# LuoGroup2023/PanTax

Measured on AMD Instinct MI355X. Metric: PAO wall-time (s) + Mreads/s: packed reads + DB (graphs and their unique-trio index) resident in HBM -> abundance tables; the metric's own GAF -> abundance quantity is value_gaf_to_tables (files -> tables, never `value`), higher is better.
Workload: dtype int64+f64

## Files before the change

### pantax_amd/csrc/api_core.cpp

```cpp
#include <algorithm>
#include <chrono>
#include <cstdio>
#include <cstdlib>
#include <cstring>
#include <memory>
#include <numeric>
#include <string>
#include "common.hpp"

using namespace ptx;

extern "C" {

int pantax_hip_db_upload(pantax_hip_ctx *ctx, const pantax_hip_graphs *g, pantax_hip_db **out) {
    if (!ctx || !g || !out) return PANTAX_HIP_E_INVALID;
    *out = nullptr;
    PTX_ENTER(ctx);
    uint32_t S = g->n_species;
    if (S == 0) return fail(ctx, PANTAX_HIP_E_INVALID, "db_upload: n_species == 0");
    std::unique_ptr<pantax_hip_db> db(new pantax_hip_db());
    db->S = S;
    if (!g->node_len) {
        std::vector<uint32_t> order(S), rs(S), re(S);
        std::iota(order.begin(), order.end(), 0u);
        std::stable_sort(order.begin(), order.end(), [&](uint32_t a, uint32_t b) { return g->range_start[a] < g->range_start[b]; });
        bool disjoint = true;
        for (uint32_t i = 0; i < S; ++i)
            if (g->range_start[i] < 0 || g->range_end[i] > 0xFFFFFFFFll) return fail(ctx, PANTAX_HIP_E_INVALID, "db_upload: species %u has an invalid node id range", i);
        for (uint32_t i = 0; i + 1 < S; ++i) if (g->range_end[order[i]] >= g->range_start[order[i + 1]]) disjoint = false;
        db->ranges_sorted_disjoint = disjoint;
        if (!disjoint) std::iota(order.begin(), order.end(), 0u);
        for (uint32_t i = 0; i < S; ++i) { rs[i] = (uint32_t)g->range_start[order[i]]; re[i] = (uint32_t)g->range_end[order[i]]; }
        db->h_range_start.assign(g->range_start, g->range_start + S);
        db->h_range_end.assign(g->range_end, g->range_end + S);
        PTX_TRY(upload(ctx, db->d_rng_start, rs.data(), S));
        PTX_TRY(upload(ctx, db->d_rng_end, re.data(), S));
        PTX_TRY(upload(ctx, db->d_rng_idx, order.data(), S));
        PTX_HIP(ctx, hipStreamSynchronize(ctx->stream));
        *out = db.release();
        return 0;
    }
// ... 196 lines not shown
        }
    }
    PTX_HIP(ctx, hipStreamSynchronize(stream));
    return 0;
}

int db_upload_finish(Ctx *ctx, pantax_hip_db *db_raw) {
    Db *const db = db_raw;
    const uint32_t S = db->S;
    const bool trace = ctx->cfg.trace;
    auto t_prev = std::chrono::steady_clock::now();
    auto lap = [&](const char *what) {
        if (!trace) return;
        (void)hipStreamSynchronize(ctx->stream);
        const auto now = std::chrono::steady_clock::now();
        std::fprintf(stderr, "[db_upload]            %-28s %9.3f ms\n", what, std::chrono::duration<double, std::milli>(now - t_prev).count());
        t_prev = now;
    };
    {
        DevBuf<uint32_t> d_flags;
        PTX_HIP(ctx, d_flags.alloc(2));
        PTX_HIP(ctx, hipMemsetAsync(d_flags.p, 0, sizeof(uint32_t), ctx->stream));
        PTX_HIP(ctx, hipMemsetAsync(d_flags.p + 1, 0xFF, sizeof(uint32_t), ctx->stream));
        PTX_TRY(node_tables_launch(ctx, db, d_flags.p));
        uint32_t fl[2] = {0, 0};
        uint64_t L = 0;
        PTX_TRY(download(ctx, fl, d_flags.p, 2));
        PTX_TRY(download(ctx, &L, db->d_bit_off.p + db->V, 1));
        PTX_TRY(download(ctx, db->h_all_same.data(), db->d_all_same.p, S));
        PTX_HIP(ctx, hipStreamSynchronize(ctx->stream));
        if (fl[0]) return fail(ctx, PANTAX_HIP_E_INVALID, "db_upload: a graph holds a node of length 0 (reference asserts > 0, profile.rs:494)");
        if (fl[1] != 0xFFFFFFFFu) return fail(ctx, PANTAX_HIP_E_INVALID, "db_upload: hap %u walks a node outside its species graph", fl[1] - 1);
        db->L = L;
        if (db->L >= NODE_REC_MAX_BITS) return fail(ctx, PANTAX_HIP_E_LIMIT, "db_upload: %llu graph bases on one GPU (limit 2^40)", (unsigned long long)db->L);
    }
    lap("node tables + checks (device)");
    {
        std::vector<uint2> tiles;
        constexpr uint64_t XCD = 8;
        for (uint32_t s = 0; s < S; ++s) {
            uint64_t maxlen = 0;
            for (uint64_t h = db->h_hap_off[s]; h < db->h_hap_off[s + 1]; ++h) maxlen = std::max<uint64_t>(maxlen, db->h_path_off[h + 1] - db->h_path_off[h]);
            const uint64_t n_chunks = (maxlen + PATH_TILE - 1) / PATH_TILE;
            for (uint64_t c0 = 0; c0 < n_chunks; c0 += XCD) {
                while (tiles.size() % XCD) tiles.push_back(make_uint2(0xFFFFFFFFu, 0u));
                for (uint64_t h = db->h_hap_off[s]; h < db->h_hap_off[s + 1]; ++h)
                    for (uint64_t c = c0; c < c0 + XCD; ++c) {
                        const bool live = c < n_chunks && c * PATH_TILE < db->h_path_off[h + 1] - db->h_path_off[h];
                        tiles.push_back(live ? make_uint2((uint32_t)h, (uint32_t)c) : make_uint2(0xFFFFFFFFu, 0u));
                    }
            }
        }
        db->n_tiles = tiles.size();
        PTX_TRY(upload(ctx, db->d_tiles, tiles.data(), tiles.size()));
        std::vector<uint32_t> hap_tile_off(db->H + 1, 0), tile_rank(tiles.size());
        for (uint64_t h = 0; h < db->H; ++h)
            hap_tile_off[h + 1] = hap_tile_off[h] + (uint32_t)((db->h_path_off[h + 1] - db->h_path_off[h] + PATH_TILE - 1) / PATH_TILE);
        for (size_t i = 0; i < tiles.size(); ++i) tile_rank[i] = tiles[i].x == 0xFFFFFFFFu ? hap_tile_off[db->H] : hap_tile_off[tiles[i].x] + tiles[i].y;
        PTX_TRY(upload(ctx, db->d_tile_rank, tile_rank.data(), tile_rank.size()));
        PTX_TRY(upload(ctx, db->d_hap_tile_off, hap_tile_off.data(), hap_tile_off.size()));
    }
    {
        const uint64_t TILE = 2048, nt = (db->V + TILE - 1) / TILE;
        std::vector<uint2> tsp(nt ? nt : 1, make_uint2(0u, 0u));
        uint32_t sp = 0;
        for (uint64_t t = 0; t < nt; ++t) {
// ... 136 lines not shown
```

### pantax_amd/csrc/common.hpp

```cpp
#pragma once
#include <hip/hip_runtime.h>
#include <cstdint>
#include <cstdio>
#include <map>
#include <functional>
#include <mutex>
#include <cstring>
#include <atomic>
#include <string>
#include <vector>
#include "../../include/pantax_hip.h"
#include "cov_state.hpp"
#include "reads_state.hpp"
#include "upload_host.hpp"

#ifndef TRIO_LH_PACK
#define TRIO_LH_PACK 0
#endif
namespace ptx {

struct Ctx;
#if TRIO_LH_PACK
using trio_len_t = uint2;
#else
// ... 255 lines not shown
    DevBuf<uint32_t> d_counts;
    uint32_t k_cap = 0;
    DevBuf<uint64_t> d_pat_mask;
    DevBuf<uint32_t> d_pat_start;
    DevBuf<uint32_t> d_pat_species;
    DevBuf<uint32_t> d_sp_pat_off;
    std::vector<uint32_t> h_sp_pat_off;
    LadPatScratch pat_scratch;
    DevBuf<double> d_x, d_x2, d_obj, d_obj2;
    DevBuf<int32_t> d_status, d_iters, d_status2, d_iters2;
    DevBuf<uint8_t> d_fixed2, d_need2;
};


struct TrioScratch {
    DevBuf<uint32_t> zero_arena;
    DevBuf<uint32_t> cnt, cursor, bucket_off, scan_tmp, first_cnt, d_tot;
    DevBuf<uint4> bucket;
    DevBuf<uint32_t> uniq_q;
    DevBuf<uint32_t> row_q;
    DevBuf<uint64_t> vis_uq;
    DevBuf<uint4> vis_rec;
    DevBuf<uint32_t> gprefix;
    uint32_t gprefix_for = 0;
    DevBuf<uint32_t> group_sums;
    DevBuf<uint32_t> hap_cnt;
};

inline uint64_t next_db_uid() { static std::atomic<uint64_t> n{1}; return n.fetch_add(1); }
struct Db {
    const uint64_t uid = next_db_uid();
    uint32_t S = 0;
    uint64_t V = 0, H = 0, P = 0, L = 0;
    std::vector<int64_t> h_range_start, h_range_end;
    std::vector<uint64_t> h_node_off, h_hap_off, h_path_off;
    bool ranges_sorted_disjoint = true;
    DevBuf<uint32_t> d_rng_start, d_rng_end, d_rng_idx;
    DevBuf<uint32_t> d_sp_first_id;
    DevBuf<uint32_t> d_node_base;
    DevBuf<uint64_t> d_bit_off;
    DevBuf<uint32_t> d_node_len;
    DevBuf<uint4> d_node_rec;
    DevBuf<uint64_t> d_path_off;
    DevBuf<uint32_t> d_path_nodes;
    DevBuf<uint32_t> d_hap_species;
    DevBuf<uint64_t> d_hap_off;
    DevBuf<uint8_t> d_all_same;
    std::vector<uint8_t> h_all_same;
    DevBuf<uint2> d_tiles;
    uint64_t n_tiles = 0;
    DevBuf<uint2> d_emit_tile_sp;
    DevBuf<uint64_t> d_node_haps;
    bool nh_built = false, nh_walk_too = false;
    DevBuf<uint32_t> d_tile_rank;
    DevBuf<uint32_t> d_hap_tile_off;
    bool trio_visit_ok = false;
    uint32_t n_vgroups = 0;
    std::vector<uint8_t> h_trio_slow;
    DevBuf<uint32_t> d_trio_slow;
    DevBuf<uint32_t> d_vis_pos;
    DevBuf<uint64_t> d_vis_head;
    DevBuf<uint32_t> d_vis_nbase;
    DevBuf<uint32_t> d_vis_sp;
    DevBuf<uint32_t> d_node_visited;
    bool trio_block_ok = false;
    uint32_t n_blocks = 0;
// ... 111 lines not shown
__host__ __device__ inline uint32_t nr_filter(uint32_t y) { return y >> 24; }
__host__ __device__ inline uint32_t nr_head(uint32_t y_old, uint32_t rows, uint32_t filter) { return (y_old & 0xFFu) | ((rows & 0xFFFFu) << 8) | (filter << 24); }
__host__ __device__ inline uint32_t nr_pair_bit(uint32_t lo, uint32_t hi) { return 1u << (((lo * 0x9E3779B1u) ^ (hi * 0x85EBCA77u)) >> 29); }
__host__ __device__ inline uint64_t nr_bit_off(const uint4 &r) { return ((uint64_t)(r.y & 0xFFu) << 32) | r.x; }
__host__ __device__ inline uint4 nr_make(uint64_t bit_off, uint32_t len) { return make_uint4((uint32_t)bit_off, (uint32_t)(bit_off >> 32) & 0xFFu, len, 0u); }

template <class T>
int upload(Ctx *ctx, DevBuf<T> &dst, const T *src, size_t n) {
    PTX_HIP(ctx, dst.alloc(n));
    if (n) PTX_HIP(ctx, hipMemcpyAsync(dst.p, src, n * sizeof(T), hipMemcpyHostToDevice, ctx->stream));
    return 0;
}
int upload_segments(Ctx *ctx, void *d_dst, const UploadSeg *segs, size_t n_segs, const std::string *files, int64_t *bad_seg, hipStream_t stream = nullptr );

constexpr uint32_t PK_BLOCK = 256, PK_UNIT = 256;
struct PackedWalks {
    uint64_t n_blocks = 0, payload_bytes = 0;
    UploadSeg first_seg, off_seg, payload_seg;
};
struct GraphPart {
    uint64_t n_nodes = 0, n_haps = 0;
    const uint64_t *path_off = nullptr;
    UploadSeg len_seg;
    bool len16 = false;
    std::vector<UploadSeg> walk_segs;
    bool packed = false;
    PackedWalks pk;
};
struct UnpackSpecies { uint32_t blk_base, off_base, payload_base , out_base, n_steps, payload_units ; };
int walks_unpack_launch(Ctx *ctx, const UnpackSpecies *d_table, uint32_t n_species, uint32_t n_blocks, const uint32_t *d_first, const uint32_t *d_off,
                        const uint8_t *d_payload, uint32_t *d_path_nodes, hipStream_t stream = nullptr );
struct WidenSpecies { uint64_t src_base , dst_base; uint64_t n; };
int lens_widen_launch(Ctx *ctx, const WidenSpecies *d_table, uint32_t n_species, uint64_t n_total, const uint16_t *d_len16, uint32_t *d_node_len, hipStream_t stream = nullptr);
int node_tables_launch(Ctx *ctx, Db *db, uint32_t *d_flags );
int db_upload_parts(Ctx *ctx, uint32_t S, const int64_t *range_start, const int64_t *range_end, const GraphPart *parts, const std::string *files,
                    pantax_hip_db **out);
int db_upload_begin(Ctx *ctx, uint32_t S, const int64_t *range_start, const int64_t *range_end, const GraphPart *parts, pantax_hip_db **out);
int db_upload_arrays(Ctx *ctx, pantax_hip_db *db, const GraphPart *parts, const std::string *files, hipStream_t stream);
int db_upload_finish(Ctx *ctx, pantax_hip_db *db);
int upload_big(Ctx *ctx, void *d_dst, const void *src, uint64_t bytes);
int upload_file(Ctx *ctx, void *d_dst, int fd, uint64_t file_off, uint64_t bytes);
int upload_text_pieces(Ctx *ctx, size_t n_pieces, void *const *d_dst, const char *text, int fd, uint64_t file_base, const uint64_t *piece_off, const uint64_t *piece_end,
                       hipStream_t stream, const std::function<bool(size_t)> &before_piece, const std::function<int(size_t)> &after_piece);
constexpr size_t PIN_UP_RING = 1u << 20, PIN_UP_MAX = 1u << 16;
template <class T>
int upload_small(Ctx *ctx, DevBuf<T> &dst, const T *src, size_t n) {
    const size_t bytes = n * sizeof(T);
    if (bytes == 0 || bytes > PIN_UP_MAX) return upload(ctx, dst, src, n);
    PTX_HIP(ctx, dst.alloc(n));
    PTX_HIP(ctx, ctx->pin_up.reserve(PIN_UP_RING));
    size_t off = (ctx->pin_up_off + 63) & ~(size_t)63;
    constexpr size_t HALF = PIN_UP_RING / 2;
    const int h_old = ctx->pin_up_off ? (int)((ctx->pin_up_off - 1) / HALF) : 0;
    if (off < HALF && off + bytes > HALF) off = HALF;
    if (off + bytes > PIN_UP_RING) off = 0;
    const int h_new = off >= HALF ? 1 : 0;
    if (h_new != h_old) {
        for (int k = 0; k < 2; ++k) {
            hipStream_t st = k == 0 ? (ctx->stream_main ? ctx->stream_main : ctx->stream) : ctx->stream2;
            if (!st) continue;
            if (!ctx->pin_up_ev[h_old][k]) PTX_HIP(ctx, hipEventCreateWithFlags(&ctx->pin_up_ev[h_old][k], hipEventDisableTiming));
            PTX_HIP(ctx, hipEventRecord(ctx->pin_up_ev[h_old][k], st));
        }
        ctx->pin_up_ev_set[h_old] = true;
        if (ctx->pin_up_ev_set[h_new])
            for (int k = 0; k < 2; ++k) if (ctx->pin_up_ev[h_new][k]) PTX_HIP(ctx, hipEventSynchronize(ctx->pin_up_ev[h_new][k]));
// ... 102 lines not shown
```

### pantax_amd/csrc/ssn_node_pass.hip

```cpp
#include <type_traits>
#include "ssn_device.hpp"

namespace ptx {

namespace {
template <bool HAPS>
__global__ void __launch_bounds__(256) ssn_hist_kernel(Sn sn) {
    __shared__ ulonglong2 tree[SN_NLEAF];
    __shared__ uint32_t s_hist[SN_NBUCKET];
    extern __shared__ unsigned long long s_dyn_tab[];
    __shared__ int s_bit[64];
    __shared__ unsigned long long s_acc[2 * 64];
    const uint32_t s = blockIdx.y, g = blockIdx.x, o = sn.node_base[s], n = sn.node_base[s + 1] - o;
    uint32_t *w = sn.w(s);
    if (n == 0 || w[SN_OFF_FLAGS] != 0) return;
    if (HAPS && sn.skip_empty && sn.hp.sp_p[s] <= 0) {
        uint32_t *row0 = sn.cntm + ((size_t)s * sn.G + g) * SN_NBUCKET;
        for (int i = threadIdx.x; i < SN_NBUCKET; i += 256) row0[i] = 0u;
        if (threadIdx.x == 0) { sn.stage_cnt[(size_t)s * sn.G + g] = 0u; if (sn.c0) sn.c0p[(size_t)s * sn.G + g] = 0.0; }
        return;
    }
    uint32_t t0, t1;
    sn_tiles(sn, n, g, t0, t1);
    const ulonglong2 *gt = reinterpret_cast<const ulonglong2 *>(w + SN_OFF_TREE);
// ... 95 lines not shown
        }
    }
    __syncthreads();
    uint32_t *row = sn.cntm + ((size_t)s * sn.G + g) * SN_NBUCKET;
    for (int i = threadIdx.x; i < SN_NBUCKET; i += 256) row[i] = s_hist[i];
    if (threadIdx.x == 0) sn.stage_cnt[(size_t)s * sn.G + g] = s_nstage;
    if (sn.c0) {
        __shared__ double s_c[4];
        cacc = wave_reduce(cacc, [](double x, double y) { return x + y; });
        if (lane == 0) s_c[threadIdx.x >> 6] = cacc;
        __syncthreads();
        if (threadIdx.x == 0) sn.c0p[(size_t)s * sn.G + g] = (s_c[0] + s_c[1]) + (s_c[2] + s_c[3]);
    }
    if (HAPS && p0 > 0 && sn.hp.ratio) {
#pragma unroll
        for (int k = 0; k < 8; ++k) {
            if (k >= p0) break;
            const unsigned long long cs = wave_reduce(c8[k], [](unsigned long long x, unsigned long long y) { return x + y; });
            const unsigned long long ls = wave_reduce(l8[k], [](unsigned long long x, unsigned long long y) { return x + y; });
            if (lane == 0) {
                if (cs) atomicAdd(&s_acc[2 * k], cs);
                if (ls) atomicAdd(&s_acc[2 * k + 1], ls);
            }
        }
        __syncthreads();
        if ((int)threadIdx.x < 2 * p0 && s_acc[threadIdx.x]) atomicAdd(&sn.hp.ratio[2 * h0 + threadIdx.x], s_acc[threadIdx.x]);
    }
}

constexpr int SN_HALF = SN_ITEMS >= 8 ? SN_ITEMS / 2 : SN_ITEMS;
static_assert(SN_ITEMS % SN_HALF == 0, "whole halves");
constexpr int SN_HALVES = SN_ITEMS / SN_HALF;
static_assert(2 * SN_HALF <= 64, "a lane per end of the half's items");
template <int NB>
__global__ void __launch_bounds__(256) node_rows_kernel(Sn sn) {
    __shared__ ulonglong2 tree[SN_NLEAF];
    __shared__ uint32_t s_hist[SN_NBUCKET];
    extern __shared__ unsigned long long s_dyn_tab[];
    __shared__ int s_bit[64];
    __shared__ unsigned long long s_acc[2 * 64];
    const uint32_t s = blockIdx.y, g = blockIdx.x, o = sn.node_base[s], n = sn.node_base[s + 1] - o;
    uint32_t *w = sn.w(s);
    if (n == 0 || w[SN_OFF_FLAGS] != 0) return;
    uint32_t t0, t1;
    sn_tiles(sn, n, g, t0, t1);
    if (sn.skip_empty && sn.hp.sp_p[s] <= 0) {
        uint32_t *row0 = sn.cntm + ((size_t)s * sn.G + g) * SN_NBUCKET;
        for (int i = threadIdx.x; i < SN_NBUCKET; i += 256) row0[i] = 0u;
        if (threadIdx.x == 0) { sn.stage_cnt[(size_t)s * sn.G + g] = 0u; if (sn.c0) sn.c0p[(size_t)s * sn.G + g] = 0.0; }
        if (!sn.fz.active || sn.fz.active[s]) {
            NodeAcc acc;
            for (uint32_t t = t0; t < t1; ++t)
#pragma unroll
                for (int r = 0; r < SN_ITEMS; ++r) {
                    const uint32_t i = t * SN_TILE + (uint32_t)r * 256u + threadIdx.x;
                    if (i < n) acc.add((double)(long long)sn.fz.bases[o + i] / (double)sn.hp.node_len[o + i], sn.fz.min_depth);
                }
            sn_block_partial<4>(acc, sn.npart + (size_t)s * sn.G + g);
        }
        return;
    }
    const ulonglong2 *gt = reinterpret_cast<const ulonglong2 *>(w + SN_OFF_TREE);
    __shared__ uint32_t s_nstage;
    const int lane = threadIdx.x & 63;
    const uint32_t wave64 = (uint32_t)__builtin_amdgcn_readfirstlane((int)(threadIdx.x >> 6)) << 6;
    constexpr int HALF = SN_HALF;
    auto end_of = [&](uint32_t q) -> uint64_t {
        const uint32_t i = q * (uint32_t)(HALF * 256) + (uint32_t)((lane >> 1) % HALF) * 256u + wave64 + (uint32_t)(lane & 1) * 64u;
        return sn.fz.bit_off[o + (i < n ? i : n)];
    };
    uint64_t endv = 0;
    if (NB && t0 < t1) endv = end_of(t0 * (uint32_t)SN_HALVES);
    for (int i = threadIdx.x; i < SN_NBUCKET; i += 256) s_hist[i] = 0;
    if (threadIdx.x == 0) s_nstage = 0;
    if (t0 < t1) for (int i = threadIdx.x; i < SN_NLEAF; i += 256) tree[i] = gt[i];
    const uint64_t h0 = sn.hp.hap_off[s], nh = sn.hp.hap_off[s + 1] - h0;
    int p0 = sn.hp.sp_p[s];
    if (p0 <= 0 || p0 > 64 || nh > 64) p0 = 0;
    const int nbyte = p0 ? (int)((nh + 7) / 8) : 0;
    if (threadIdx.x < 64) s_bit[threadIdx.x] = (p0 && threadIdx.x < nh) ? sn.hp.hap_bit[h0 + threadIdx.x] : -1;
    if (threadIdx.x < 128) s_acc[threadIdx.x] = 0;
    __syncthreads();
    for (int b = 0; b < nbyte; ++b) {
        unsigned long long e = 0ull;
#pragma unroll
        for (int i = 0; i < 8; ++i) { const int bit = s_bit[8 * b + i]; if (((threadIdx.x >> i) & 1u) && bit >= 0) e |= 1ull << bit; }
        s_dyn_tab[b * 256 + threadIdx.x] = e;
    }
    __syncthreads();
    uint64_t eb[2 * HALF];
#pragma unroll
    for (int k = 0; k < 2 * HALF; ++k) eb[k] = NB ? lane_get(endv, k) : 0ull;
    unsigned long long c8[8] = {0, 0, 0, 0, 0, 0, 0, 0}, l8[8] = {0, 0, 0, 0, 0, 0, 0, 0};
    const uint32_t stage0 = o + t0 * SN_TILE;
    double cacc = 0.0;
    NodeAcc nacc;
    static_assert((uint64_t)SN_TILE * sizeof(unsigned long long) < (1ull << 20), "a lane's byte offset from the half's base: 32 bits with room to spare");
    auto half = [&](auto guard, const uint32_t t, const int hb) __attribute__((always_inline)) {
        constexpr bool GUARD = decltype(guard)::value;
        __builtin_amdgcn_sched_barrier(0);
        const uint32_t hbase = t * SN_TILE + (uint32_t)hb * 256u, base = hbase + threadIdx.x;
        double av[HALF];
        uint64_t mv[HALF];
        uint32_t cv[HALF], lv[HALF];
        {
            unsigned long long bs[HALF];
            uint32_t fw[HALF];
            uint64_t gb[HALF];
            uint32_t bw0[HALF], bw1[HALF];
            bool fits[HALF];
            uint32_t nwv[HALF], tbv[HALF];
            if (NB) {
#pragma unroll
                for (int r = 0; r < HALF; ++r) {
                    const uint64_t b0 = eb[2 * r], b1 = eb[2 * r + 1], w0 = b0 >> 5;
                    const uint32_t nw = b1 > b0 ? (uint32_t)(((b1 - 1) >> 5) - w0) + 1u : 0u, cap = 64u * (uint32_t)NB;
                    gb[r] = b0;
                    nwv[r] = nw;
                    tbv[r] = (uint32_t)(b1 - b0);
                    fits[r] = nw <= cap && !NRK_ABL(1u);
                    const uint32_t top = nw ? (nw < cap ? nw : cap) - 1u : 0u;
                    const uint32_t *wp = sn.fz.bitmap + (nw ? w0 : 0ull);
                    bw0[r] = wp[(uint32_t)lane < top ? (uint32_t)lane : top];
                    bw1[r] = NB > 1 ? wp[(uint32_t)lane + 64u < top ? (uint32_t)lane + 64u : top] : 0u;
                }
                endv = end_of(t * (uint32_t)SN_HALVES + (uint32_t)(hb / HALF) + 1u);
                __builtin_amdgcn_sched_barrier(0);
            }
#pragma unroll
            for (int r = 0; r < HALF; ++r) {
                if constexpr (GUARD) {
                    const uint32_t i = base + (uint32_t)r * 256u;
// ... 63 lines not shown
                    const uint32_t ce = sl - (uint32_t)__popc(wl & ~(0xFFFFFFFFu >> (31u - ((fe - 1u) & 31u))));
                    const uint32_t e = j0 >= nw ? ce : px + (uint32_t)__popc(x & ((1u << (f0 & 31u)) - 1u));
                    const uint32_t cc = wave_shl1(e, ce) - e;
                    if (count) c = cc;
                } else if (count) {
                    const uint64_t g0 = gb[r] + exr, g1 = g0 + lv[r], w0 = g0 >> 5, w1 = (g1 - 1) >> 5;
                    const uint32_t m0 = 0xFFFFFFFFu << (g0 & 31), m1 = 0xFFFFFFFFu >> (31 - (uint32_t)((g1 - 1) & 31));
                    c = w0 == w1 ? __popc(bw0[r] & m0 & m1) : __popc(bw0[r] & m0) + __popc(bw1[r] & m1);
                    for (uint64_t ww = w0 + 1; ww < w1; ++ww) c += __popc(sn.fz.bitmap[ww]);
                }
                cv[r] = c;
                av[r] = 0.0;
                if (!GUARD || i < n) {
                    av[r] = (double)(long long)bs[r] / (double)lv[r];
                    nacc.add(av[r], sn.fz.min_depth);
                }
                if constexpr (!GUARD) __builtin_amdgcn_sched_barrier(0);
            }
        }
        [[maybe_unused]] uint32_t idv[HALF];
#ifndef NODE_ROWS_SERIAL_DESCENT
        {
            uint64_t ka[HALF];
#pragma unroll
            for (int r = 0; r < HALF; ++r) ka[r] = (uint64_t)__double_as_longlong(av[r]);
            if (NRK_ABL(2u)) {
#pragma unroll
                for (int r = 0; r < HALF; ++r) idv[r] = 2u * ((uint32_t)(ka[r] >> 30) & (uint32_t)(SN_NLEAF - 1));
            } else sn_bucket_ids<HALF>(tree, mv, ka, idv);
        }
#endif
#pragma unroll
        for (int r = 0; r < HALF; ++r) {
            {
                const unsigned long long m = mv[r];
                if (m) {
                    const unsigned long long c = cv[r], l = lv[r];
#pragma unroll
                    for (int k = 0; k < 8; ++k)
                        if (k < p0) { const bool on = (m >> k) & 1ull; c8[k] += on ? c : 0ull; l8[k] += on ? l : 0ull; }
                    unsigned long long rest = m >> 8;
                    while (rest) {
                        const int k = __ffsll((long long)rest) - 1 + 8;
                        rest &= rest - 1;
                        if (c) atomicAdd(&s_acc[2 * k], c);
                        atomicAdd(&s_acc[2 * k + 1], l);
                    }
                }
            }
            uint32_t id = SN_NO_ROW;
            const uint64_t abits = (uint64_t)__double_as_longlong(av[r]);
            if (av[r] > 0.0 && mv[r] == 0ull) cacc += av[r];
            if (av[r] > 0.0 && mv[r] != 0ull) {
#ifdef NODE_ROWS_SERIAL_DESCENT
                const Key2 key{mv[r], abits};
                uint32_t k = 1;
                if (NRK_ABL(2u)) k = (uint32_t)SN_NLEAF + ((uint32_t)(abits >> 30) & (uint32_t)(SN_NLEAF - 1));
                else
#pragma unroll
                for (int l = 0; l < SN_LEVELS; ++l) { const ulonglong2 nd = tree[k]; k = 2u * k + (less2(Key2{nd.x, nd.y}, key) ? 1u : 0u); }
                const uint32_t lo = k - (uint32_t)SN_NLEAF;
                uint32_t eq = 0;
                if (lo < (uint32_t)SN_NSPLIT && !NRK_ABL(2u)) { const ulonglong2 nd = tree[tree_node(lo)]; eq = eq2(Key2{nd.x, nd.y}, key) ? 1u : 0u; }
                id = 2u * lo + eq;
#else
                id = idv[r];
#endif
                atomicAdd(&s_hist[id], 1u);
            }
            const bool travels = id != SN_NO_ROW && !(id & 1u);
            const unsigned long long bal = __ballot(travels);
            if (bal) {
                uint32_t wbase = 0;
                if (lane == 0) wbase = atomicAdd(&s_nstage, (uint32_t)__popcll(bal));
                wbase = (uint32_t)__builtin_amdgcn_readfirstlane((int)wbase);
                if (travels) {
                    const uint32_t pos = stage0 + wbase + (uint32_t)__popcll(bal & ((1ull << lane) - 1ull));
                    sn.stage[pos] = make_ulonglong2(mv[r], abits);
                    sn.ids[pos] = (uint16_t)id;
                }
            }
        }
    };
    const uint32_t tf = n / SN_TILE < t1 ? n / SN_TILE : t1;
    for (uint32_t t = t0; t < tf; ++t) {
#pragma unroll
        for (int hb = 0; hb < SN_ITEMS; hb += HALF) half(std::false_type{}, t, hb);
    }
    if (t0 < t1 && tf < t1) {
#pragma unroll
        for (int hb = 0; hb < SN_ITEMS; hb += HALF) half(std::true_type{}, tf, hb);
    }
    __syncthreads();
    sn_block_partial<4>(nacc, sn.npart + (size_t)s * sn.G + g);
    uint32_t *row = sn.cntm + ((size_t)s * sn.G + g) * SN_NBUCKET;
    for (int i = threadIdx.x; i < SN_NBUCKET; i += 256) row[i] = s_hist[i];
    if (threadIdx.x == 0) sn.stage_cnt[(size_t)s * sn.G + g] = s_nstage;
    if (sn.c0) {
        __shared__ double s_c[4];
        cacc = wave_reduce(cacc, [](double x, double y) { return x + y; });
        if (lane == 0) s_c[threadIdx.x >> 6] = cacc;
        __syncthreads();
        if (threadIdx.x == 0) sn.c0p[(size_t)s * sn.G + g] = (s_c[0] + s_c[1]) + (s_c[2] + s_c[3]);
    }
    if (p0 > 0 && sn.hp.ratio) {
#pragma unroll
        for (int k = 0; k < 8; ++k) {
            if (k >= p0) break;
            const unsigned long long cs = wave_reduce(c8[k], [](unsigned long long x, unsigned long long y) { return x + y; });
            const unsigned long long ls = wave_reduce(l8[k], [](unsigned long long x, unsigned long long y) { return x + y; });
            if (lane == 0) {
                if (cs) atomicAdd(&s_acc[2 * k], cs);
                if (ls) atomicAdd(&s_acc[2 * k + 1], ls);
            }
        }
        __syncthreads();
        if ((int)threadIdx.x < 2 * p0 && s_acc[threadIdx.x]) atomicAdd(&sn.hp.ratio[2 * h0 + threadIdx.x], s_acc[threadIdx.x]);
    }
}

__global__ void __launch_bounds__(64) node_rows_final_kernel(Sn sn) {
    const uint32_t s = blockIdx.x, n = sn.node_base[s + 1] - sn.node_base[s];
    double mx = -INFINITY, zs = 0.0; unsigned long long nv = 0, zc = 0;
    if (n != 0 && sn.fz.active && !sn.fz.active[s]) mx = 0.0;
    else if (n != 0) {
        const uint32_t nt = (n + SN_TILE - 1) / SN_TILE, ng = n <= (uint32_t)SN_SAMPLE ? 1u : (nt + sn.per - 1) / sn.per;
        for (uint32_t g = threadIdx.x; g < ng; g += 64) { const NodePartial p = sn.npart[(size_t)s * sn.G + g]; mx = fmax(mx, p.mx); zs += p.zs; nv += p.nv; zc += p.zc; }
    }
    mx = wave_reduce(mx, [](double x, double y) { return fmax(x, y); });
    zs = wave_reduce(zs, [](double x, double y) { return x + y; });
    nv = wave_reduce(nv, [](unsigned long long x, unsigned long long y) { return x + y; });
    zc = wave_reduce(zc, [](unsigned long long x, unsigned long long y) { return x + y; });
    if (threadIdx.x == 0) { sn.fz.amax[s] = mx; sn.fz.nvalid[s] = (uint32_t)nv; sn.fz.nzsum[s] = zs; sn.fz.nzcnt[s] = (uint32_t)zc; }
}
}

void ssn_node_rows_launch(Ctx *ctx, const Sn &sn, uint32_t S, uint32_t max_haps, int node_bits) {
    const size_t lds = (size_t)((max_haps + 7) / 8) * 256 * sizeof(unsigned long long);
    if (node_bits == 0) hipLaunchKernelGGL(node_rows_kernel<0>, dim3(sn.G, S), dim3(256), lds, ctx->stream, sn);
    else if (node_bits == 1) hipLaunchKernelGGL(node_rows_kernel<1>, dim3(sn.G, S), dim3(256), lds, ctx->stream, sn);
    else hipLaunchKernelGGL(node_rows_kernel<2>, dim3(sn.G, S), dim3(256), lds, ctx->stream, sn);
    hipLaunchKernelGGL(node_rows_final_kernel, dim3(S), dim3(64), 0, ctx->stream, sn);
}
// ... 8 lines not shown
```

### pantax_amd/csrc/ssn_plan.hpp

```cpp
#pragma once
#include <cstddef>
#include <cstdint>

namespace ptx {

#ifndef SN_LEVELS
#define SN_LEVELS 10
#endif
constexpr int SN_SAMPLE = 4096;
constexpr int SN_NLEAF = 1 << SN_LEVELS;
constexpr int SN_NBUCKET = 2 * SN_NLEAF;
#ifndef SN_ITEMS_N
#define SN_ITEMS_N 8
#endif
constexpr int SN_ITEMS = SN_ITEMS_N;
constexpr int SN_TILE = 256 * SN_ITEMS;
constexpr uint32_t SN_TARGET_WGS = 8192;
constexpr uint32_t SN_TIE_ROWS = 8192;
#ifndef SN_HEAD_PAIRS
#define SN_HEAD_PAIRS 64
#endif
constexpr int SN_HP = SN_HEAD_PAIRS, SN_NWH = SN_NLEAF / SN_HP;
constexpr bool SSN_TIES_ASYNC_AUTO = false;
constexpr uint64_t SSN_MAX_SEG = 1ull << 26;

constexpr size_t SN_OFF_FLAGS = 0;
constexpr size_t SN_OFF_TREE = 4;
constexpr size_t SN_OFF_SAMP = SN_OFF_TREE + 4 * SN_NLEAF;
constexpr size_t SN_OFF_START = SN_OFF_SAMP + 2 * 2 * SN_SAMPLE;
constexpr size_t SN_OFF_MED = SN_OFF_START + SN_NBUCKET + 4;
constexpr size_t SN_OFF_BIG = SN_OFF_MED + SN_NBUCKET;
constexpr size_t SN_WS_WORDS = SN_OFF_BIG + SN_NBUCKET;
static_assert(SN_WS_WORDS % 4 == 0, "16-byte tree nodes");

constexpr size_t SN_NODE_PARTIAL_WORDS = 8;

struct SsnPlan {
    uint32_t G = 1, per = 1;
    uint32_t tie_grid = 1;
    size_t ws = 0;
    size_t cntm = 0;
    size_t stage_cnt = 0;
    size_t c0p = 0;
    size_t seg_n = 0;
    size_t seg_out = 0;
    size_t sub_k = 0;
    size_t ids = 0;
    size_t npart = 0;
    size_t total_words = 0;
};
SsnPlan ssn_plan(uint32_t S, uint64_t seg_bound, uint64_t V);

int ssn_keys_all(const char *option, bool has_patterns);
constexpr int SSN_NODE_BITS_WORDS = 2;
int ssn_node_bits(const char *option, int words);
bool ssn_ties_async(int option, bool clocked, bool on_side_stream, bool have_side_stream);

}
```

### pantax_amd/csrc/stage_db.hip

```cpp
#include <memory>
#include "common.hpp"
#include "primitives.hpp"
#include "wave.hpp"

namespace ptx {

namespace {
constexpr int NT_PER = 16, NT_TILE = 256 * NT_PER;

__global__ void __launch_bounds__(256) node_len_tile_sum_kernel(const uint32_t *__restrict__ len, uint64_t V, unsigned long long *__restrict__ sums,
                                                                uint32_t *__restrict__ zero_flag) {
    __shared__ unsigned long long s_w[4];
    const uint64_t base = (uint64_t)blockIdx.x * NT_TILE;
    unsigned long long c = 0;
    bool zero = false;
#pragma unroll
    for (int k = 0; k < NT_PER; ++k) {
        const uint64_t i = base + (uint64_t)k * 256 + threadIdx.x;
        if (i < V) { const uint32_t l = len[i]; c += l; zero = zero || l == 0u; }
    }
    if (__any(zero) && (threadIdx.x & 63) == 0) *zero_flag = 1u;
    c = wave_reduce(c, [](unsigned long long x, unsigned long long y) { return x + y; });
    if ((threadIdx.x & 63) == 0) s_w[threadIdx.x >> 6] = c;
    __syncthreads();
// ... 20 lines not shown
        if (i < n_tiles) sums[i] = carry + woff + incl - v;
        __syncthreads();
        if (threadIdx.x == 0) s_carry = carry + tot;
        __syncthreads();
    }
    if (threadIdx.x == 0) sums[n_tiles] = s_carry;
}
__global__ void __launch_bounds__(256) node_tables_kernel(const uint32_t *__restrict__ len, uint64_t V, const unsigned long long *__restrict__ sums,
                                                          uint64_t *__restrict__ bit_off, uint4 *__restrict__ node_rec) {
    __shared__ unsigned long long s_w[2][4];
    const uint64_t base = (uint64_t)blockIdx.x * NT_TILE;
    const uint32_t lane = threadIdx.x & 63, wave = threadIdx.x >> 6;
    unsigned long long run = sums[blockIdx.x];
#pragma unroll 4
    for (int k = 0; k < NT_PER; ++k) {
        const uint64_t i = base + (uint64_t)k * 256 + threadIdx.x;
        const uint32_t l = i < V ? len[i] : 0u;
        unsigned long long incl = l;
#pragma unroll
        for (int d = 1; d < 64; d <<= 1) { const unsigned long long t = __shfl_up(incl, d); if (lane >= (uint32_t)d) incl += t; }
        if (lane == 63) s_w[k & 1][wave] = incl;
        __syncthreads();
        unsigned long long woff = 0, tot = 0;
#pragma unroll
        for (int w = 0; w < 4; ++w) { const unsigned long long t = s_w[k & 1][w]; woff += w < (int)wave ? t : 0ull; tot += t; }
        if (i < V) {
            const unsigned long long bo = run + woff + (incl - l);
            bit_off[i] = bo;
            node_rec[i] = nr_make(bo, l);
        }
        run += tot;
    }
    if (blockIdx.x == gridDim.x - 1 && threadIdx.x == 0) bit_off[V] = sums[gridDim.x];
}

__global__ void __launch_bounds__(256) walk_check_kernel(const uint64_t *__restrict__ path_off, const uint32_t *__restrict__ path_nodes,
                                                         const uint32_t *__restrict__ hap_species, const uint32_t *__restrict__ node_base,
                                                         uint32_t *__restrict__ bad ) {
    const uint32_t h = blockIdx.x;
    const uint32_t s = hap_species[h];
    const uint32_t nv = node_base[s + 1] - node_base[s];
    uint32_t mx = 0;
    for (uint64_t q = path_off[h] + threadIdx.x; q < path_off[h + 1]; q += 256) mx = max(mx, path_nodes[q]);
    mx = wave_reduce(mx, [](uint32_t x, uint32_t y) { return x > y ? x : y; });
    if ((threadIdx.x & 63) == 0 && path_off[h + 1] > path_off[h] && mx >= nv) atomicMin(bad, h + 1);
}

__global__ void __launch_bounds__(256) walks_same_kernel(const uint64_t *__restrict__ path_off, const uint32_t *__restrict__ path_nodes,
                                                         const uint32_t *__restrict__ hap_species, const uint64_t *__restrict__ hap_off,
                                                         uint8_t *__restrict__ all_same) {
    const uint32_t h = blockIdx.x, s = hap_species[h];
    const uint64_t h0 = hap_off[s];
    if (h == h0) return;
    const uint64_t a0 = path_off[h0], a1 = path_off[h0 + 1], b0 = path_off[h], b1 = path_off[h + 1];
    if (a1 - a0 != b1 - b0) { if (threadIdx.x == 0) all_same[s] = 0; return; }
    for (uint64_t q = 0; q < a1 - a0; q += 256) {
        const uint64_t i = q + threadIdx.x;
        const bool diff = i < a1 - a0 && path_nodes[a0 + i] != path_nodes[b0 + i];
        if (__syncthreads_or(diff)) { if (threadIdx.x == 0) all_same[s] = 0; return; }
    }
}

__global__ void __launch_bounds__(256) walks_unpack_kernel(const UnpackSpecies *__restrict__ table, uint32_t n_species, uint32_t n_blocks, const uint32_t *__restrict__ first,
                                                           const uint32_t *__restrict__ off, const uint8_t *__restrict__ payload, uint32_t *__restrict__ out) {
    const int lane = threadIdx.x & 63;
    const uint32_t gb = (uint32_t)__builtin_amdgcn_readfirstlane((int)(blockIdx.x * 4u + (threadIdx.x >> 6)));
// ... 24 lines not shown
                                                         uint32_t *__restrict__ dst) {
    const int lane = threadIdx.x & 63;
    const uint64_t e0 = ((uint64_t)blockIdx.x * 4 + (threadIdx.x >> 6)) * 1024;
    if (e0 >= n_total) return;
    uint32_t lo = 0, hi = n_species - 1;
    while (lo < hi) { const uint32_t mid = (lo + hi + 1) >> 1; if (table[mid].src_base <= e0 + (uint64_t)lane) lo = mid; else hi = mid - 1; }
    uint32_t s = lo;
    for (uint32_t r = 0; r < 16; ++r) {
        const uint64_t i = e0 + (uint64_t)r * 64 + (uint64_t)lane;
        if (i >= n_total) break;
        while (s + 1 < n_species && table[s + 1].src_base <= i) ++s;
        const uint64_t k = i - table[s].src_base;
        if (k < table[s].n) dst[table[s].dst_base + k] = (uint32_t)src[i];
    }
}
}

int walks_unpack_launch(Ctx *ctx, const UnpackSpecies *d_table, uint32_t n_species, uint32_t n_blocks, const uint32_t *d_first, const uint32_t *d_off,
                        const uint8_t *d_payload, uint32_t *d_path_nodes, hipStream_t stream) {
    if (!n_blocks || !n_species) return 0;
    std::unique_ptr<KTimer> t(stream ? nullptr : new KTimer(ctx, "walks_unpack_kernel"));
    hipLaunchKernelGGL(walks_unpack_kernel, dim3((n_blocks + 3) / 4), dim3(256), 0, stream ? stream : ctx->stream, d_table, n_species, n_blocks, d_first, d_off, d_payload, d_path_nodes);
    PTX_HIP(ctx, hipGetLastError());
    return 0;
}
int lens_widen_launch(Ctx *ctx, const WidenSpecies *d_table, uint32_t n_species, uint64_t n_total, const uint16_t *d_len16, uint32_t *d_node_len, hipStream_t stream) {
    if (!n_total || !n_species) return 0;
    std::unique_ptr<KTimer> t(stream ? nullptr : new KTimer(ctx, "lens_widen_kernel"));
    hipLaunchKernelGGL(lens_widen_kernel, dim3((uint32_t)((n_total + 4095) / 4096)), dim3(256), 0, stream ? stream : ctx->stream, d_table, n_species, n_total, d_len16, d_node_len);
    PTX_HIP(ctx, hipGetLastError());
    return 0;
}

int node_tables_launch(Ctx *ctx, Db *db, uint32_t *d_flags) {
    const uint64_t V = db->V;
    const uint32_t n_tiles = (uint32_t)((V + NT_TILE - 1) / NT_TILE);
    DevBuf<unsigned long long> sums;
    PTX_HIP(ctx, sums.alloc((size_t)n_tiles + 1));
    if (n_tiles) {
        hipLaunchKernelGGL(node_len_tile_sum_kernel, dim3(n_tiles), dim3(256), 0, ctx->stream, (const uint32_t *)db->d_node_len.p, V, sums.p, d_flags);
        hipLaunchKernelGGL(u64_scan_kernel, dim3(1), dim3(1024), 0, ctx->stream, sums.p, n_tiles);
        hipLaunchKernelGGL(node_tables_kernel, dim3(n_tiles), dim3(256), 0, ctx->stream, (const uint32_t *)db->d_node_len.p, V, (const unsigned long long *)sums.p,
                           db->d_bit_off.p, db->d_node_rec.p);
    } else PTX_HIP(ctx, hipMemsetAsync(db->d_bit_off.p, 0, sizeof(uint64_t), ctx->stream));
    if (db->H) {
        hipLaunchKernelGGL(walk_check_kernel, dim3((uint32_t)db->H), dim3(256), 0, ctx->stream, db->d_path_off.p, db->d_path_nodes.p,
                           db->d_hap_species.p, db->d_node_base.p, d_flags + 1);
        hipLaunchKernelGGL(walks_same_kernel, dim3((uint32_t)db->H), dim3(256), 0, ctx->stream, db->d_path_off.p, db->d_path_nodes.p,
                           db->d_hap_species.p, db->d_hap_off.p, db->d_all_same.p);
    }
    PTX_HIP(ctx, hipGetLastError());
    PTX_HIP(ctx, hipStreamSynchronize(ctx->stream));
    return 0;
}

}
```

### pantax_amd/csrc/stage_lp_rows.hip

```cpp
#include <algorithm>
#include <cstdio>
#include <vector>
#include "lad.hpp"
#include "lad_device.hpp"
#include "cov_plan.hpp"
#include "primitives.hpp"
#include "wave.hpp"
#include "scan_chained.hpp"

namespace ptx {

__device__ __forceinline__ uint32_t find_hap_l(const uint64_t *__restrict__ path_off, uint32_t H, uint64_t q) {
    uint32_t lo = 0, hi = H;
    while (lo < hi) { uint32_t mid = (lo + hi) >> 1; if (path_off[mid] <= q) lo = mid + 1; else hi = mid; }
    return lo - 1;
}

__global__ void __launch_bounds__(256) mask_kernel(const uint2 *__restrict__ tiles, const uint64_t *__restrict__ path_off,
                                                   const uint32_t *__restrict__ path_nodes, const uint32_t *__restrict__ hap_species,
                                                   const uint32_t *__restrict__ node_base, const int32_t *__restrict__ hap_bit,
                                                   unsigned long long *__restrict__ mask, const int32_t *__restrict__ sp_p,
                                                   const uint32_t *__restrict__ wide_off ,
                                                   const uint32_t *__restrict__ wide_nw, unsigned long long *__restrict__ maskw,
                                                   const uint64_t *__restrict__ by_node_hap_off ) {
    const uint2 tile = tiles[blockIdx.x];
    if (tile.x == 0xFFFFFFFFu) return;
    const uint32_t h = tile.x;
    const int bit = hap_bit[h];
    if (bit < 0) return;
    const uint32_t sp = hap_species[h];
    const uint32_t nb = node_base[sp];
    const uint64_t q0 = path_off[h] + (uint64_t)tile.y * PATH_TILE, qend = path_off[h + 1];
    if (wide_off && sp_p[sp] > LAD_MAXP) {
        const unsigned long long m = 1ull << (bit & 63);
        const size_t nw = wide_nw[sp];
        unsigned long long *base = maskw + (size_t)wide_off[sp] * LAD_WIDE_NW + (bit >> 6);
        for (uint64_t q = q0 + threadIdx.x; q < q0 + PATH_TILE && q < qend; q += 256) {
            unsigned long long *w = base + (size_t)path_nodes[q] * nw;
// ... 418 lines not shown
    for (uint32_t s_ = 0; s_ < S; ++s_) {
        r.max_vs = std::max<uint64_t>(r.max_vs, db->h_node_off[s_ + 1] - db->h_node_off[s_]);
        max_hs = std::max<uint64_t>(max_hs, db->h_hap_off[s_ + 1] - db->h_hap_off[s_]);
    }
    r.max_haps = (uint32_t)max_hs;
    r.use_nodes = V > SS_MAX_N && r.max_vs <= SSN_MAX_SEG && S <= 65535;
    if (!ctx->cfg.row_sort.empty()) {
        const char *ev = ctx->cfg.row_sort.c_str();
        if (ev[0] == 'r') r.use_nodes = false;
        if (ev[0] == 'n') r.use_nodes = r.max_vs <= SSN_MAX_SEG && S <= 65535 && V > 0;
    }
    r.use_sample = V <= SS_MAX_N;
    r.by_node = use_node_haps(ctx, db);
    r.ratio_by_node = r.by_node && V && !ctx->cfg.ratio_kernel;
    r.wide = max_hs > (uint64_t)LAD_MAXP;
    const bool mask_pass_env = ctx->cfg.mask_pass || ctx->cfg.objective == "nodes";
    r.masks_in_sort = r.use_nodes && r.ratio_by_node && !db->nh_walk_too && !r.wide && !mask_pass_env;
    return r;
}
int row_pack_shift(const RowRoute &rt, uint32_t S, int pmax_bound) {
    const int sp_bits = S > 1 ? bits_for(S - 1) : 0;
    return (!rt.use_sample && sp_bits + pmax_bound <= 64 && !(rt.use_nodes && pmax_bound >= 64)) ? pmax_bound : -1;
}

LadShape lad_shape(const std::string &option, uint32_t n_workgroups, int n_cu, int pmax_bound) {
    if (pmax_bound > 16 || option == "roomy") return LadShape::roomy;
    if (option == "compact") return LadShape::compact;
    return n_workgroups > (uint32_t)std::max(n_cu, 0) ? LadShape::compact : LadShape::roomy;
}
const char *lad_shape_name(LadShape s) { return s == LadShape::compact ? "compact" : "roomy"; }

bool node_pass_fused_eligible(const Ctx *ctx, const Db *db, const pantax_hip_strain_config *cfg, bool readers_clean) {
    if (ctx->cfg.node_pass == "split" || !db->cov.count_pending() || db->V == 0) return false;
    if (cfg->sample_nodes != 0 || ctx->cfg.cov_readers_clean || readers_clean) return false;
    if (long_node_shape(db->L, db->V, ctx->cfg.ncs_prefix_min, ctx->cfg.ncs_no_prefix)) return false;
    return row_route(ctx, db).masks_in_sort;
}

static int upload_candidates(Ctx *ctx, const Db *db, LadBatch *lb) {
    const uint32_t S = db->S;
    const uint64_t H = db->H;
    std::vector<int32_t> hap_bit(H ? H : 1, -1);
    for (uint32_t s = 0; s < S; ++s)
        for (int k = 0; k < lb->h_p[s]; ++k) hap_bit[db->h_hap_off[s] + lb->h_cand[db->h_hap_off[s] + k]] = k;
    PTX_TRY(upload(ctx, lb->d_hap_bit, hap_bit.data(), hap_bit.size()));
    PTX_TRY(upload(ctx, lb->d_p, lb->h_p.data(), S));
    return 0;
}
static int wide_layout(Ctx *ctx, const Db *db, LadBatch *lb, const RowRoute &rt) {
    const uint32_t S = db->S;
    if (!lb->wide_laid_out) {
        std::vector<uint32_t> off(S ? S : 1, 0xFFFFFFFFu), slot(S ? S : 1, 0xFFFFFFFFu), nwv(S ? S : 1, 0u), list;
        std::vector<uint64_t> woff, coff;
        uint64_t vw = 0, wtot = 0, ctot = 0;
        uint32_t n_huge = 0;
        for (uint32_t s = 0; s < S; ++s) {
            const uint64_t Hs = db->h_hap_off[s + 1] - db->h_hap_off[s];
            if (Hs <= (uint64_t)LAD_MAXP) continue;
            if (Hs > 30000ull) return fail(ctx, PANTAX_HIP_E_LIMIT, "lad_prepare: species %u has %llu haplotypes; the basis inverse is indexed with 32 bits (30000 columns)", s, (unsigned long long)Hs);
            const uint32_t nw = (uint32_t)((Hs + LAD_WIDEP - 1) / LAD_WIDEP) * LAD_WIDE_NW;
            off[s] = (uint32_t)vw; slot[s] = (uint32_t)list.size(); list.push_back(s); nwv[s] = nw;
            vw += (db->h_node_off[s + 1] - db->h_node_off[s]) * (nw / LAD_WIDE_NW);
            woff.push_back(wtot); coff.push_back(ctot);
            wtot += 64ull * nw * 64ull * nw;
            if (nw > (uint32_t)LAD_WIDE_NW) { ++n_huge; ctot += 64ull * nw; }
        }
// ... 171 lines not shown
```

Measured before the change: 7299.

## Pack per-column count/length sums into one u64 and specialise column count

The node_rows kernel's per-column accumulators for count and length are merged into a single 64-bit packed value, halving the accumulator registers. The kernel body is also instantiated per compile-time column count, taken from the species' candidate count, so unused columns and the overflow atomic path are compiled out. To keep the packed 32-bit fields safe, db_upload now computes the largest per-species base count on the device and downloads it, and the fused node pass is disabled when that count exceeds 32 bits. This adds a small kernel plus a synchronising download at upload time, and more kernel instantiations.

```diff
diff --git a/pantax_amd/csrc/api_core.cpp b/pantax_amd/csrc/api_core.cpp
--- a/pantax_amd/csrc/api_core.cpp
+++ b/pantax_amd/csrc/api_core.cpp
@@ -7,6 +7,7 @@
 #include <numeric>
 #include <string>
 #include "common.hpp"
+#include "ssn_plan.hpp"
 
 using namespace ptx;
 
@@ -269,6 +270,9 @@
         if (fl[0]) return fail(ctx, PANTAX_HIP_E_INVALID, "db_upload: a graph holds a node of length 0 (reference asserts > 0, profile.rs:494)");
         if (fl[1] != 0xFFFFFFFFu) return fail(ctx, PANTAX_HIP_E_INVALID, "db_upload: hap %u walks a node outside its species graph", fl[1] - 1);
         db->L = L;
+        std::vector<uint64_t> ends;
+        PTX_TRY(species_ends_download(ctx, db, ends));
+        db->max_species_bases = ssn_max_species_bases(ends.data(), S);
         if (db->L >= NODE_REC_MAX_BITS) return fail(ctx, PANTAX_HIP_E_LIMIT, "db_upload: %llu graph bases on one GPU (limit 2^40)", (unsigned long long)db->L);
     }
     lap("node tables + checks (device)");
diff --git a/pantax_amd/csrc/common.hpp b/pantax_amd/csrc/common.hpp
--- a/pantax_amd/csrc/common.hpp
+++ b/pantax_amd/csrc/common.hpp
@@ -311,6 +311,7 @@
     const uint64_t uid = next_db_uid();
     uint32_t S = 0;
     uint64_t V = 0, H = 0, P = 0, L = 0;
+    uint64_t max_species_bases = 0;
     std::vector<int64_t> h_range_start, h_range_end;
     std::vector<uint64_t> h_node_off, h_hap_off, h_path_off;
     bool ranges_sorted_disjoint = true;
@@ -488,6 +489,7 @@
                         const uint8_t *d_payload, uint32_t *d_path_nodes, hipStream_t stream = nullptr );
 struct WidenSpecies { uint64_t src_base , dst_base; uint64_t n; };
 int lens_widen_launch(Ctx *ctx, const WidenSpecies *d_table, uint32_t n_species, uint64_t n_total, const uint16_t *d_len16, uint32_t *d_node_len, hipStream_t stream = nullptr);
+int species_ends_download(Ctx *ctx, Db *db, std::vector<uint64_t> &ends );
 int node_tables_launch(Ctx *ctx, Db *db, uint32_t *d_flags );
 int db_upload_parts(Ctx *ctx, uint32_t S, const int64_t *range_start, const int64_t *range_end, const GraphPart *parts, const std::string *files,
                     pantax_hip_db **out);
diff --git a/pantax_amd/csrc/ssn_node_pass.hip b/pantax_amd/csrc/ssn_node_pass.hip
--- a/pantax_amd/csrc/ssn_node_pass.hip
+++ b/pantax_amd/csrc/ssn_node_pass.hip
@@ -151,6 +151,27 @@
 static_assert(SN_ITEMS % SN_HALF == 0, "whole halves");
 constexpr int SN_HALVES = SN_ITEMS / SN_HALF;
 static_assert(2 * SN_HALF <= 64, "a lane per end of the half's items");
+#ifndef NODE_ROWS_SUMS_UNPACKED
+struct ColSum {
+    uint64_t v = 0;
+    __device__ __forceinline__ void add(bool on, uint32_t c, uint32_t l) { v = sn_packed_add(v, on, sn_packed(c, l)); }
+    __device__ __forceinline__ uint64_t c() const { return sn_packed_c(v); }
+    __device__ __forceinline__ uint64_t l() const { return sn_packed_l(v); }
+};
+#else
+struct ColSum {
+    uint64_t cs = 0, ls = 0;
+    __device__ __forceinline__ void add(bool on, uint32_t c, uint32_t l) { cs += on ? (uint64_t)c : 0ull; ls += on ? (uint64_t)l : 0ull; }
+    __device__ __forceinline__ uint64_t c() const { return cs; }
+    __device__ __forceinline__ uint64_t l() const { return ls; }
+};
+#endif
+template <int K, class F>
+__device__ __forceinline__ void sn_for_columns(int nc, F &&f) {
+    if constexpr (K >= 8) f(std::integral_constant<int, 8>{});
+    else if (nc <= K) f(std::integral_constant<int, K>{});
+    else sn_for_columns<K + SN_NC_STEP>(nc, f);
+}
 template <int NB>
 __global__ void __launch_bounds__(256) node_rows_kernel(Sn sn) {
     __shared__ ulonglong2 tree[SN_NLEAF];
@@ -210,13 +231,14 @@
     uint64_t eb[2 * HALF];
 #pragma unroll
     for (int k = 0; k < 2 * HALF; ++k) eb[k] = NB ? lane_get(endv, k) : 0ull;
-    unsigned long long c8[8] = {0, 0, 0, 0, 0, 0, 0, 0}, l8[8] = {0, 0, 0, 0, 0, 0, 0, 0};
+    ColSum c8[8];
     const uint32_t stage0 = o + t0 * SN_TILE;
     double cacc = 0.0;
     NodeAcc nacc;
     static_assert((uint64_t)SN_TILE * sizeof(unsigned long long) < (1ull << 20), "a lane's byte offset from the half's base: 32 bits with room to spare");
-    auto half = [&](auto guard, const uint32_t t, const int hb) __attribute__((always_inline)) {
+    auto half = [&](auto guard, auto nc, const uint32_t t, const int hb) __attribute__((always_inline)) {
         constexpr bool GUARD = decltype(guard)::value;
+        [[maybe_unused]] constexpr int NC = decltype(nc)::value;
         __builtin_amdgcn_sched_barrier(0);
         const uint32_t hbase = t * SN_TILE + (uint32_t)hb * 256u, base = hbase + threadIdx.x;
         double av[HALF];
@@ -346,19 +368,24 @@
 #endif
 #pragma unroll
         for (int r = 0; r < HALF; ++r) {
-            {
+            if constexpr (NC > 0) {
                 const unsigned long long m = mv[r];
                 if (m) {
-                    const unsigned long long c = cv[r], l = lv[r];
-#pragma unroll
-                    for (int k = 0; k < 8; ++k)
-                        if (k < p0) { const bool on = (m >> k) & 1ull; c8[k] += on ? c : 0ull; l8[k] += on ? l : 0ull; }
-                    unsigned long long rest = m >> 8;
-                    while (rest) {
-                        const int k = __ffsll((long long)rest) - 1 + 8;
-                        rest &= rest - 1;
-                        if (c) atomicAdd(&s_acc[2 * k], c);
-                        atomicAdd(&s_acc[2 * k + 1], l);
+                    const uint32_t c = cv[r], l = lv[r];
+#pragma unroll
+                    for (int k = 0; k < NC; ++k)
+#ifdef NODE_ROWS_NC_RUNTIME
+                        if (k < p0)
+#endif
+                        c8[k].add((m >> k) & 1ull, c, l);
+                    if constexpr (NC == 8) {
+                        unsigned long long rest = m >> 8;
+                        while (rest) {
+                            const int k = __ffsll((long long)rest) - 1 + 8;
+                            rest &= rest - 1;
+                            if (c) atomicAdd(&s_acc[2 * k], (unsigned long long)c);
+                            atomicAdd(&s_acc[2 * k + 1], (unsigned long long)l);
+                        }
                     }
                 }
             }
@@ -397,14 +424,21 @@
         }
     };
     const uint32_t tf = n / SN_TILE < t1 ? n / SN_TILE : t1;
-    for (uint32_t t = t0; t < tf; ++t) {
-#pragma unroll
-        for (int hb = 0; hb < SN_ITEMS; hb += HALF) half(std::false_type{}, t, hb);
-    }
-    if (t0 < t1 && tf < t1) {
-#pragma unroll
-        for (int hb = 0; hb < SN_ITEMS; hb += HALF) half(std::true_type{}, tf, hb);
-    }
+    auto tiles = [&](auto nc) __attribute__((always_inline)) {
+        for (uint32_t t = t0; t < tf; ++t) {
+#pragma unroll
+            for (int hb = 0; hb < SN_ITEMS; hb += HALF) half(std::false_type{}, nc, t, hb);
+        }
+        if (t0 < t1 && tf < t1) {
+#pragma unroll
+            for (int hb = 0; hb < SN_ITEMS; hb += HALF) half(std::true_type{}, nc, tf, hb);
+        }
+    };
+#ifdef NODE_ROWS_NC_RUNTIME
+    tiles(std::integral_constant<int, 8>{});
+#else
+    sn_for_columns<0>(ssn_body_columns(p0), tiles);
+#endif
     __syncthreads();
     sn_block_partial<4>(nacc, sn.npart + (size_t)s * sn.G + g);
     uint32_t *row = sn.cntm + ((size_t)s * sn.G + g) * SN_NBUCKET;
@@ -421,8 +455,8 @@
 #pragma unroll
         for (int k = 0; k < 8; ++k) {
             if (k >= p0) break;
-            const unsigned long long cs = wave_reduce(c8[k], [](unsigned long long x, unsigned long long y) { return x + y; });
-            const unsigned long long ls = wave_reduce(l8[k], [](unsigned long long x, unsigned long long y) { return x + y; });
+            const unsigned long long cs = wave_reduce((unsigned long long)c8[k].c(), [](unsigned long long x, unsigned long long y) { return x + y; });
+            const unsigned long long ls = wave_reduce((unsigned long long)c8[k].l(), [](unsigned long long x, unsigned long long y) { return x + y; });
             if (lane == 0) {
                 if (cs) atomicAdd(&s_acc[2 * k], cs);
                 if (ls) atomicAdd(&s_acc[2 * k + 1], ls);
diff --git a/pantax_amd/csrc/ssn_plan.hpp b/pantax_amd/csrc/ssn_plan.hpp
--- a/pantax_amd/csrc/ssn_plan.hpp
+++ b/pantax_amd/csrc/ssn_plan.hpp
@@ -54,6 +54,29 @@
 int ssn_keys_all(const char *option, bool has_patterns);
 constexpr int SSN_NODE_BITS_WORDS = 2;
 int ssn_node_bits(const char *option, int words);
+#ifdef __HIPCC__
+#define SN_HD __host__ __device__
+#else
+#define SN_HD
+#endif
+constexpr uint64_t SN_PACKED_FIELD_MAX = 0xFFFFFFFFull;
+SN_HD inline uint64_t sn_packed(uint32_t c, uint32_t l) { return ((uint64_t)c << 32) | (uint64_t)l; }
+SN_HD inline uint64_t sn_packed_add(uint64_t acc, bool on, uint64_t cl) { return acc + (on ? cl : 0ull); }
+SN_HD inline uint64_t sn_packed_c(uint64_t acc) { return acc >> 32; }
+SN_HD inline uint64_t sn_packed_l(uint64_t acc) { return acc & 0xFFFFFFFFull; }
+inline bool ssn_packed_sums_fit(uint64_t max_species_bases) { return max_species_bases <= SN_PACKED_FIELD_MAX; }
+inline uint64_t ssn_max_species_bases(const uint64_t *ends, uint32_t S) {
+    uint64_t mx = 0;
+    for (uint32_t s = 0; s < S; ++s) if (ends[s + 1] - ends[s] > mx) mx = ends[s + 1] - ends[s];
+    return mx;
+}
+#ifndef NODE_ROWS_NC_STEP
+#define NODE_ROWS_NC_STEP 1
+#endif
+constexpr int SN_NC_STEP = NODE_ROWS_NC_STEP;
+static_assert(SN_NC_STEP == 1 || SN_NC_STEP == 2 || SN_NC_STEP == 4 || SN_NC_STEP == 8, "the register columns are whole steps");
+SN_HD constexpr int ssn_body_columns(int p) { return p <= 0 ? 0 : p >= 8 ? 8 : (p + SN_NC_STEP - 1) / SN_NC_STEP * SN_NC_STEP; }
+
 bool ssn_ties_async(int option, bool clocked, bool on_side_stream, bool have_side_stream);
 
 }
diff --git a/pantax_amd/csrc/stage_db.hip b/pantax_amd/csrc/stage_db.hip
--- a/pantax_amd/csrc/stage_db.hip
+++ b/pantax_amd/csrc/stage_db.hip
@@ -76,6 +76,11 @@
         run += tot;
     }
     if (blockIdx.x == gridDim.x - 1 && threadIdx.x == 0) bit_off[V] = sums[gridDim.x];
+}
+
+__global__ void __launch_bounds__(256) species_ends_kernel(const uint32_t *__restrict__ node_base, const uint64_t *__restrict__ bit_off, uint32_t S, uint64_t *__restrict__ ends) {
+    const uint32_t s = blockIdx.x * 256u + threadIdx.x;
+    if (s <= S) ends[s] = bit_off[node_base[s]];
 }
 
 __global__ void __launch_bounds__(256) walk_check_kernel(const uint64_t *__restrict__ path_off, const uint32_t *__restrict__ path_nodes,
@@ -166,6 +171,18 @@
     return 0;
 }
 
+int species_ends_download(Ctx *ctx, Db *db, std::vector<uint64_t> &ends) {
+    const uint32_t S = db->S;
+    DevBuf<uint64_t> d_ends;
+    PTX_HIP(ctx, d_ends.alloc((size_t)S + 1));
+    hipLaunchKernelGGL(species_ends_kernel, dim3(S / 256 + 1), dim3(256), 0, ctx->stream, (const uint32_t *)db->d_node_base.p, (const uint64_t *)db->d_bit_off.p, S, d_ends.p);
+    PTX_HIP(ctx, hipGetLastError());
+    ends.assign((size_t)S + 1, 0);
+    PTX_TRY(download(ctx, ends.data(), d_ends.p, (size_t)S + 1));
+    PTX_HIP(ctx, hipStreamSynchronize(ctx->stream));
+    return 0;
+}
+
 int node_tables_launch(Ctx *ctx, Db *db, uint32_t *d_flags) {
     const uint64_t V = db->V;
     const uint32_t n_tiles = (uint32_t)((V + NT_TILE - 1) / NT_TILE);
diff --git a/pantax_amd/csrc/stage_lp_rows.hip b/pantax_amd/csrc/stage_lp_rows.hip
--- a/pantax_amd/csrc/stage_lp_rows.hip
+++ b/pantax_amd/csrc/stage_lp_rows.hip
@@ -4,6 +4,7 @@
 #include "lad.hpp"
 #include "lad_device.hpp"
 #include "cov_plan.hpp"
+#include "ssn_plan.hpp"
 #include "primitives.hpp"
 #include "wave.hpp"
 #include "scan_chained.hpp"
@@ -488,6 +489,7 @@
 
 bool node_pass_fused_eligible(const Ctx *ctx, const Db *db, const pantax_hip_strain_config *cfg, bool readers_clean) {
     if (ctx->cfg.node_pass == "split" || !db->cov.count_pending() || db->V == 0) return false;
+    if (!ssn_packed_sums_fit(db->max_species_bases)) return false;
     if (cfg->sample_nodes != 0 || ctx->cfg.cov_readers_clean || readers_clean) return false;
     if (long_node_shape(db->L, db->V, ctx->cfg.ncs_prefix_min, ctx->cfg.ncs_no_prefix)) return false;
     return row_route(ctx, db).masks_in_sort;
```

After: 7375 (median of 4 runs). 1.0% higher.
